# daigo0927/tf-raft

Measured on NVIDIA H100. Metric: frame-pairs/sec at 448×512 iters=12; final-flow max-abs vs ref, higher is better.
Workload: dtype f32

## Files before the change

tf_raft_b200/csrc/kernels.cuh:

```cuda
#pragma once
#include "common.cuh"

namespace raft {

__global__ void split_plane_kernel(const float* __restrict__ src, int src_stride, int src_c0, int nch, int nch_pad,
                                   __half* __restrict__ hi, __half* __restrict__ lo, int dst_stride, int dst_c0,
                                   size_t npix, float scale) {
  const size_t total = npix * (size_t)nch_pad;
  for (size_t i = blockIdx.x * (size_t)blockDim.x + threadIdx.x; i < total; i += (size_t)gridDim.x * blockDim.x) {
    const size_t px = i / nch_pad;
    const int c = (int)(i - px * nch_pad);
    __half h = __float2half_rn(0.f), l = h;
    if (c < nch) split_f16(src[px * src_stride + src_c0 + c] * scale, h, l);
    hi[px * dst_stride + dst_c0 + c] = h;
    lo[px * dst_stride + dst_c0 + c] = l;
  }
}

__global__ void avgpool2x2_kernel(const float* __restrict__ src, float* __restrict__ dst, size_t M, int H, int W,
                                  int C) {
  const int Ho = H / 2, Wo = W / 2;
  const size_t total = M * (size_t)Ho * Wo * C;
  for (size_t i = blockIdx.x * (size_t)blockDim.x + threadIdx.x; i < total; i += (size_t)gridDim.x * blockDim.x) {
    size_t t = i;
    const int c = (int)(t % C);
    t /= C;
    const int xo = (int)(t % Wo);
    t /= Wo;
    const int yo = (int)(t % Ho);
    const size_t m = t / Ho;
    const float* s = src + ((m * H + 2 * yo) * W + 2 * xo) * (size_t)C + c;
    const float a = s[0], b = s[C], cc = s[(size_t)W * C], d = s[(size_t)W * C + C];
    dst[i] = __fmul_rn(__fadd_rn(__fadd_rn(a, b), __fadd_rn(cc, d)), 0.25f);
  }
}

__global__ void coords_grid_kernel(float* __restrict__ out, int B, int h, int w) {
  const size_t total = (size_t)B * h * w;
  for (size_t i = blockIdx.x * (size_t)blockDim.x + threadIdx.x; i < total; i += (size_t)gridDim.x * blockDim.x) {
    const int x = (int)(i % w), y = (int)((i / w) % h);
    out[2 * i] = (float)x;
    out[2 * i + 1] = (float)y;
  }
}

struct TapGather { float c00, c01, c10, c11; int o00, o01, o10, o11; };
__device__ __forceinline__ TapGather tap_setup(int H, int W, float px, float py) {
  const float gx = fminf(fmaxf(px, 0.0f), (float)(W - 1));
  const float gy = fminf(fmaxf(py, 0.0f), (float)(H - 1));
  const float gx0 = floorf(gx), gx1 = ceilf(gx), gy0 = floorf(gy), gy1 = ceilf(gy);
  const float wy1 = __fsub_rn(gy1, gy), wy0 = __fsub_rn(gy, gy0);
  const float wx1 = __fsub_rn(gx1, gx), wx0 = __fsub_rn(gx, gx0);
  TapGather t;
  t.c00 = __fmul_rn(wy1, wx1); t.c01 = __fmul_rn(wy1, wx0);
  t.c10 = __fmul_rn(wy0, wx1); t.c11 = __fmul_rn(wy0, wx0);
  const int ix0 = (int)gx0, ix1 = (int)gx1, iy0 = (int)gy0, iy1 = (int)gy1;
  t.o00 = iy0 * W + ix0; t.o01 = iy0 * W + ix1; t.o10 = iy1 * W + ix0; t.o11 = iy1 * W + ix1;
  return t;
}
__device__ __forceinline__ float tap_combine(const TapGather& t, float x00, float x01, float x10, float x11) {
  float acc = __fmul_rn(t.c00, x00);
  acc = __fadd_rn(acc, __fmul_rn(t.c01, x01));
  acc = __fadd_rn(acc, __fmul_rn(t.c10, x10));
  acc = __fadd_rn(acc, __fmul_rn(t.c11, x11));
  return acc;
}
__device__ __forceinline__ float sample_floor_ceil(const float* __restrict__ img, int H, int W, float px, float py) {
  const TapGather t = tap_setup(H, W, px, py);
  return tap_combine(t, __ldg(img + t.o00), __ldg(img + t.o01), __ldg(img + t.o10), __ldg(img + t.o11));
}

__global__ void bilinear_sampler_kernel(const float* __restrict__ image, const float* __restrict__ coords, int M, int H,
                                        int W, int P, float* __restrict__ out) {
  const size_t total = (size_t)M * P;
  for (size_t i = blockIdx.x * (size_t)blockDim.x + threadIdx.x; i < total; i += (size_t)gridDim.x * blockDim.x) {
    const size_t m = i / P;
    out[i] = sample_floor_ceil(image + m * (size_t)H * W, H, W, coords[2 * i], coords[2 * i + 1]);
  }
}

struct LookupParams {
  const float* pyr[RAFT_MAX_LEVELS];
  int lh[RAFT_MAX_LEVELS], lw[RAFT_MAX_LEVELS];
  const float* coords;
  float* out; int out_stride;
  __half* out_hi; __half* out_lo; int h_stride, h_pad;
  int nq;
  int levels, radius;
  const float* im_flow; __half* im_hi; __half* im_lo; int im_B, im_h, im_w;
};

__global__ void __launch_bounds__(256) corr_lookup_kernel(const LookupParams p) {
  __shared__ float4 axis_smem[8 * 32];
  const int warps_per_block = blockDim.x >> 5;
  const int lane = threadIdx.x & 31;
  const int side = 2 * p.radius + 1, ntap = side * side;
  const size_t nwork = (size_t)p.nq * p.levels;
  for (size_t wi = (size_t)blockIdx.x * warps_per_block + (threadIdx.x >> 5); wi < nwork;
       wi += (size_t)gridDim.x * warps_per_block) {
    const int q = (int)(wi / p.levels), l = (int)(wi % p.levels);
    const int H = p.lh[l], W = p.lw[l];
    const float* img = p.pyr[l] + (size_t)q * H * W;
    const float inv = 1.0f / (float)(1 << l);
    const float cx = __fmul_rn(__ldg(p.coords + 2 * (size_t)q), inv);
    const float cy = __fmul_rn(__ldg(p.coords + 2 * (size_t)q + 1), inv);
    constexpr int kMaxIter = 3;
    if (ntap <= 32 * kMaxIter && side <= 16) {
      float4* ax = axis_smem + (threadIdx.x >> 5) * 32;
      __syncwarp();
      if (lane < 2 * side) {
        const bool isy = lane >= side;
        const int i = isy ? lane - side : lane;
        const float cc = isy ? cy : cx;
        const int dim = isy ? H : W;
        const float g = fminf(fmaxf(__fadd_rn(cc, (float)(i - p.radius)), 0.0f), (float)(dim - 1));
        const float g0 = floorf(g), g1 = ceilf(g);
        ax[(isy ? 16 : 0) + i] = make_float4(__fsub_rn(g1, g), __fsub_rn(g, g0), __int_as_float((int)g0), __int_as_float((int)g1));
      }
      __syncwarp();
      TapGather tg[kMaxIter];
      float x00[kMaxIter], x01[kMaxIter], x10[kMaxIter], x11[kMaxIter];
#pragma unroll
      for (int i = 0; i < kMaxIter; ++i) {
        const int t = min(lane + 32 * i, ntap - 1);
        const int a = t / side, b2 = t - a * side;
        const float4 sx = ax[a], sy = ax[16 + b2];
        const int ix0 = __float_as_int(sx.z), ix1 = __float_as_int(sx.w), iy0 = __float_as_int(sy.z), iy1 = __float_as_int(sy.w);
        tg[i].c00 = __fmul_rn(sy.x, sx.x); tg[i].c01 = __fmul_rn(sy.x, sx.y);
        tg[i].c10 = __fmul_rn(sy.y, sx.x); tg[i].c11 = __fmul_rn(sy.y, sx.y);
        x00[i] = __ldg(img + iy0 * W + ix0); x01[i] = __ldg(img + iy0 * W + ix1);
        x10[i] = __ldg(img + iy1 * W + ix0); x11[i] = __ldg(img + iy1 * W + ix1);
      }
#pragma unroll
      for (int i = 0; i < kMaxIter; ++i) {
        const int t = lane + 32 * i;
        if (t < ntap) {
          const float v = tap_combine(tg[i], x00[i], x01[i], x10[i], x11[i]);
          const int ch = l * ntap + t;
          if (p.out) p.out[(size_t)q * p.out_stride + ch] = v;
          if (p.out_hi) {
            __half hh, ll;
            split_f16(v, hh, ll);
            p.out_hi[(size_t)q * p.h_stride + ch] = hh;
            p.out_lo[(size_t)q * p.h_stride + ch] = ll;
          }
        }
      }
    } else {
      for (int t = lane; t < ntap; t += 32) {
        const int a = t / side, b2 = t - a * side;
        const float px = __fadd_rn(cx, (float)(a - p.radius));
        const float py = __fadd_rn(cy, (float)(b2 - p.radius));
        const float v = sample_floor_ceil(img, H, W, px, py);
        const int ch = l * ntap + t;
        if (p.out) p.out[(size_t)q * p.out_stride + ch] = v;
        if (p.out_hi) {
          __half hh, ll;
          split_f16(v, hh, ll);
          p.out_hi[(size_t)q * p.h_stride + ch] = hh;
          p.out_lo[(size_t)q * p.h_stride + ch] = ll;
        }
      }
    }
    if (p.out_hi && l == p.levels - 1) {
      const __half zero = __float2half_rn(0.f);
      for (int c = p.levels * ntap + lane; c < p.h_pad; c += 32) {
        p.out_hi[(size_t)q * p.h_stride + c] = zero;
        p.out_lo[(size_t)q * p.h_stride + c] = zero;
      }
    }
  }
}

__global__ void __launch_bounds__(256) corr_fp32_kernel(const float* __restrict__ f1, const float* __restrict__ f2,
                                                        float* __restrict__ out, int N, int C, float div) {
  __shared__ float As[16][64 + 4];
  __shared__ float Bs[16][64 + 4];
  const int b = blockIdx.z;
  const float* A = f1 + (size_t)b * N * C;
  const float* Bm = f2 + (size_t)b * N * C;
  float* O = out + (size_t)b * N * N;
  const int m0 = blockIdx.y * 64, n0 = blockIdx.x * 64;
  const int tx = threadIdx.x & 15, ty = threadIdx.x >> 4;
  const int lr = threadIdx.x >> 2, lc = (threadIdx.x & 3) * 4;
  float acc[4][4] = {};
  for (int k0 = 0; k0 < C; k0 += 16) {
#pragma unroll
    for (int j = 0; j < 4; ++j) {
      const int k = k0 + lc + j;
      As[lc + j][lr] = (m0 + lr < N && k < C) ? A[(size_t)(m0 + lr) * C + k] : 0.f;
      Bs[lc + j][lr] = (n0 + lr < N && k < C) ? Bm[(size_t)(n0 + lr) * C + k] : 0.f;
    }
    __syncthreads();
#pragma unroll
    for (int k = 0; k < 16; ++k) {
      float a[4], w[4];
#pragma unroll
      for (int i = 0; i < 4; ++i) {
        a[i] = As[k][ty * 4 + i];
        w[i] = Bs[k][tx * 4 + i];
      }
#pragma unroll
      for (int i = 0; i < 4; ++i)
#pragma unroll
        for (int j = 0; j < 4; ++j) acc[i][j] = fmaf(a[i], w[j], acc[i][j]);
    }
    __syncthreads();
  }
#pragma unroll
  for (int i = 0; i < 4; ++i)
#pragma unroll
    for (int j = 0; j < 4; ++j) {
      const int m = m0 + ty * 4 + i, n = n0 + tx * 4 + j;
      if (m < N && n < N) O[(size_t)m * N + n] = __fdiv_rn(acc[i][j], div);
    }
}

enum SimtAct : int { SACT_NONE = 0, SACT_RELU = 1, SACT_SIGMOID = 2, SACT_TANH = 3 };

struct SimtConvParams {
  const float* src[3]; int src_stride[3], src_c0[3], src_n[3]; int nsrc;
  const float* w; const float* bias;
  int kh, kw, cin, cout;
  int B, H, W;
  int stride, Hin, Win, pad_t, pad_l;
  int in_image_norm;
  const float* post_scale; const float* post_shift;
  float* out; int out_stride, out_c0;
  __half* out_hi; __half* out_lo; int h_stride, h_c0;
  int act; float out_scale;
};

__global__ void __launch_bounds__(256) conv_simt_kernel(const SimtConvParams p) {
  __shared__ float As[16][64 + 4];
  __shared__ float Ws[16][64 + 4];
  const int npix = p.B * p.H * p.W;
  const int m0 = blockIdx.x * 64, n0 = blockIdx.y * 64;
  const int tx = threadIdx.x & 15, ty = threadIdx.x >> 4;
  const int lr = threadIdx.x >> 2, lc = (threadIdx.x & 3) * 4;
  const int wr = threadIdx.x >> 4, wc = (threadIdx.x & 15) * 4;
  const int st = p.stride > 1 ? p.stride : 1;
  const int Hin = p.stride > 0 ? p.Hin : p.H, Win = p.stride > 0 ? p.Win : p.W;
  const int ph = p.stride > 0 ? p.pad_t : (p.kh - 1) / 2, pw = p.stride > 0 ? p.pad_l : (p.kw - 1) / 2;
  const int lp = m0 + lr;
  int lb = 0, ly = 0, lx = 0;
  if (lp < npix) {
    lx = lp % p.W;
    ly = (lp / p.W) % p.H;
    lb = lp / (p.W * p.H);
  }
  float acc[4][4] = {};
  for (int tap = 0; tap < p.kh * p.kw; ++tap) {
    const int dy = tap / p.kw - ph, dx = tap % p.kw - pw;
    const int sy = ly * st + dy, sx = lx * st + dx;
    const bool inb = lp < npix && sy >= 0 && sy < Hin && sx >= 0 && sx < Win;
    const size_t spix = ((size_t)lb * Hin + (inb ? sy : 0)) * Win + (inb ? sx : 0);
    for (int k0 = 0; k0 < p.cin; k0 += 16) {
#pragma unroll
      for (int j = 0; j < 4; ++j) {
        const int c = k0 + lc + j;
        float v = 0.f;
        if (inb && c < p.cin) {
          int cc = c, s = 0;
          while (s < p.nsrc - 1 && cc >= p.src_n[s]) cc -= p.src_n[s++];
          v = __ldg(p.src[s] + spix * p.src_stride[s] + p.src_c0[s] + cc);
          if (p.in_image_norm) v = __fsub_rn(__fmul_rn(2.0f, __fdiv_rn(v, 255.0f)), 1.0f);
        }
        As[lc + j][lr] = v;
      }
      {
        const int c = k0 + wr;
#pragma unroll
        for (int j = 0; j < 4; ++j) {
          const int n = n0 + wc + j;
          Ws[wr][wc + j] = (c < p.cin && n < p.cout) ? __ldg(p.w + ((size_t)tap * p.cin + c) * p.cout + n) : 0.f;
        }
      }
      __syncthreads();
#pragma unroll
      for (int k = 0; k < 16; ++k) {
        float a[4], w[4];
#pragma unroll
        for (int i = 0; i < 4; ++i) {
          a[i] = As[k][ty * 4 + i];
          w[i] = Ws[k][tx * 4 + i];
        }
#pragma unroll
        for (int i = 0; i < 4; ++i)
#pragma unroll
          for (int j = 0; j < 4; ++j) acc[i][j] = fmaf(a[i], w[j], acc[i][j]);
      }
      __syncthreads();
    }
  }
#pragma unroll
  for (int i = 0; i < 4; ++i) {
    const int m = m0 + ty * 4 + i;
    if (m >= npix) continue;
#pragma unroll
    for (int j = 0; j < 4; ++j) {
      const int n = n0 + tx * 4 + j;
      if (n >= p.cout) continue;
      float v = acc[i][j] + (p.bias ? __ldg(p.bias + n) : 0.f);
      if (p.post_scale) v = v * __ldg(p.post_scale + n) + __ldg(p.post_shift + n);
      if (p.act == SACT_RELU) v = relu_nan(v);
      else if (p.act == SACT_SIGMOID) v = sigmoidf_acc(v);
      else if (p.act == SACT_TANH) v = tanhf(v);
      v *= p.out_scale;
      if (p.out) p.out[(size_t)m * p.out_stride + p.out_c0 + n] = v;
      if (p.out_hi) {
        __half hh, ll;
        split_f16(v, hh, ll);
        p.out_hi[(size_t)m * p.h_stride + p.h_c0 + n] = hh;
        p.out_lo[(size_t)m * p.h_stride + p.h_c0 + n] = ll;
      }
    }
  }
}

__global__ void gru_rh_kernel(const float* __restrict__ r, const float* __restrict__ h, float* __restrict__ rh,
                              size_t n) {
  for (size_t i = blockIdx.x * (size_t)blockDim.x + threadIdx.x; i < n; i += (size_t)gridDim.x * blockDim.x)
    rh[i] = r[i] * h[i];
}
__global__ void gru_update_kernel(const float* __restrict__ z, const float* __restrict__ q, float* __restrict__ h,
                                  size_t n) {
  for (size_t i = blockIdx.x * (size_t)blockDim.x + threadIdx.x; i < n; i += (size_t)gridDim.x * blockDim.x)
    h[i] = (1.0f - z[i]) * h[i] + z[i] * q[i];
}

__global__ void copy_channels_kernel(const float* __restrict__ src, int src_stride, int src_c0,
                                     float* __restrict__ dst, int dst_stride, int dst_c0, int n, size_t npix) {
  const size_t total = npix * (size_t)n;
  for (size_t i = blockIdx.x * (size_t)blockDim.x + threadIdx.x; i < total; i += (size_t)gridDim.x * blockDim.x) {
    const size_t px = i / n;
    const int c = (int)(i - px * n);
    dst[px * dst_stride + dst_c0 + c] = src[px * src_stride + src_c0 + c];
  }
}

__global__ void flow_advance_kernel(float* __restrict__ coords1, const float* __restrict__ delta,
                                    float* __restrict__ flow, int B, int h, int w) {
  const size_t total = (size_t)B * h * w;
  for (size_t i = blockIdx.x * (size_t)blockDim.x + threadIdx.x; i < total; i += (size_t)gridDim.x * blockDim.x) {
    const float gx = (float)(i % w), gy = (float)((i / w) % h);
    float cx = coords1[2 * i], cy = coords1[2 * i + 1];
    if (delta) {
      cx = __fadd_rn(cx, delta[2 * i]);
      cy = __fadd_rn(cy, delta[2 * i + 1]);
      coords1[2 * i] = cx;
      coords1[2 * i + 1] = cy;
    }
    flow[2 * i] = __fsub_rn(cx, gx);
    flow[2 * i + 1] = __fsub_rn(cy, gy);
  }
}

__global__ void __launch_bounds__(256) upsample_convex_kernel(const float* __restrict__ flow,
                                                              const float* __restrict__ mask, int B, int h, int w,
                                                              float* __restrict__ out) {
  const int sub = threadIdx.x & 63;
  const size_t npix = (size_t)B * h * w;
  for (size_t pix = (size_t)blockIdx.x * 4 + (threadIdx.x >> 6); pix < npix; pix += (size_t)gridDim.x * 4) {
    const int x = (int)(pix % w), y = (int)((pix / w) % h), b = (int)(pix / ((size_t)w * h));
    const float* mp = mask + pix * 576 + sub * 9;
    float m[9], mx = -INFINITY;
#pragma unroll
    for (int k = 0; k < 9; ++k) {
      m[k] = __ldg(mp + k);
      mx = fmaxf(mx, m[k]);
    }
    float sum = 0.f;
#pragma unroll
    for (int k = 0; k < 9; ++k) {
      m[k] = expf(m[k] - mx);
      sum += m[k];
    }
    float ox = 0.f, oy = 0.f;
#pragma unroll
    for (int k = 0; k < 9; ++k) {
      const int yy = y + k / 3 - 1, xx = x + k % 3 - 1;
      float fx = 0.f, fy = 0.f;
      if (yy >= 0 && yy < h && xx >= 0 && xx < w) {
        const float* fp = flow + (((size_t)b * h + yy) * w + xx) * 2;
        fx = 8.0f * __ldg(fp);
        fy = 8.0f * __ldg(fp + 1);
      }
      const float wk = m[k] / sum;
      ox += wk * fx;
      oy += wk * fy;
    }
    const int by = sub >> 3, bx = sub & 7;
    float* op = out + ((((size_t)b * 8 * h) + 8 * y + by) * (8 * (size_t)w) + 8 * x + bx) * 2;
    *reinterpret_cast<float2*>(op) = make_float2(ox, oy);
  }
}

__global__ void upflow8_kernel(const float* __restrict__ flow, int B, int h, int w, float* __restrict__ out) {
  const int H = 8 * h, W = 8 * w;
  const size_t total = (size_t)B * H * W;
  for (size_t i = blockIdx.x * (size_t)blockDim.x + threadIdx.x; i < total; i += (size_t)gridDim.x * blockDim.x) {
    const int X = (int)(i % W), Y = (int)((i / W) % H), b = (int)(i / ((size_t)W * H));
    const float sx = ((float)X + 0.5f) * 0.125f - 0.5f, sy = ((float)Y + 0.5f) * 0.125f - 0.5f;
    const float fx0 = floorf(sx), fy0 = floorf(sy);
    const float ax = sx - fx0, ay = sy - fy0;
    const int x0 = min(max((int)fx0, 0), w - 1), x1 = min(max((int)fx0 + 1, 0), w - 1);
    const int y0 = min(max((int)fy0, 0), h - 1), y1 = min(max((int)fy0 + 1, 0), h - 1);
    const float* f = flow + (size_t)b * h * w * 2;
#pragma unroll
    for (int c = 0; c < 2; ++c) {
      const float v00 = f[((size_t)y0 * w + x0) * 2 + c], v01 = f[((size_t)y0 * w + x1) * 2 + c];
      const float v10 = f[((size_t)y1 * w + x0) * 2 + c], v11 = f[((size_t)y1 * w + x1) * 2 + c];
      const float top = v00 * (1.f - ax) + v01 * ax, bot = v10 * (1.f - ax) + v11 * ax;
      out[2 * i + c] = 8.0f * (top * (1.f - ay) + bot * ay);
    }
  }
}

__global__ void absmax_kernel(const float* __restrict__ w, size_t n, unsigned int* __restrict__ out_bits) {
  float m = 0.f;
  for (size_t i = blockIdx.x * (size_t)blockDim.x + threadIdx.x; i < n; i += (size_t)gridDim.x * blockDim.x)
    m = fmaxf(m, fabsf(w[i]));
  for (int o = 16; o > 0; o >>= 1) m = fmaxf(m, __shfl_xor_sync(0xffffffffu, m, o));
  if ((threadIdx.x & 31) == 0) atomicMax(out_bits, __float_as_uint(m));
}

__global__ void weight_scale_kernel(const unsigned int* __restrict__ absmax_bits, float* __restrict__ scale) {
  const float m = __uint_as_float(*absmax_bits);
  int k = 0;
  if (m > 0.f && isfinite(m)) {
    int e;
    frexpf(m, &e);
    k = 13 - e;
    k = max(-24, min(24, k));
  }
  scale[0] = ldexpf(1.0f, k);
  scale[1] = ldexpf(1.0f, -k);
}

struct PackParams {
  const float* w; int kh, kw, cin, cout;
  __half* hi; __half* lo; int cout_pad, cin_pad, cout_off;
  int r_src0[2], r_n[2], r_dst0[2], nrange;
  const float* scale;
};
__global__ void pack_weights_kernel(const PackParams p) {
  const size_t total = (size_t)p.kh * p.kw * p.cin * p.cout;
  const float s = p.scale[0];
  for (size_t i = blockIdx.x * (size_t)blockDim.x + threadIdx.x; i < total; i += (size_t)gridDim.x * blockDim.x) {
    size_t t = i;
    const int n = (int)(t % p.cout);
    t /= p.cout;
    const int c = (int)(t % p.cin);
    const int tap = (int)(t / p.cin);
    int cd = -1;
    for (int r = 0; r < p.nrange; ++r)
      if (c >= p.r_src0[r] && c < p.r_src0[r] + p.r_n[r]) cd = p.r_dst0[r] + (c - p.r_src0[r]);
    if (cd < 0) continue;
    __half hh, ll;
    split_f16(p.w[i] * s, hh, ll);
    const size_t o = ((size_t)tap * p.cout_pad + p.cout_off + n) * p.cin_pad + cd;
    p.hi[o] = hh;
    p.lo[o] = ll;
  }
}

constexpr int kNormBlock = 8;
__device__ __forceinline__ void chan_merge(float& na, float& ma, float& m2a, float nb, float mb, float m2b) {
  if (nb == 0.f) return;
  const float n = na + nb, d = mb - ma;
  ma = ma + d * (nb / n);
  m2a = m2a + m2b + d * d * (na * nb / n);
  na = n;
}
__global__ void __launch_bounds__(256) norm_stats_kernel(const float* __restrict__ y, int P, int C, int nsplit,
                                                         float* __restrict__ part) {
  __shared__ float red[3][256];
  const int g = blockIdx.x, sp = blockIdx.y;
  const int lanes = 256 / C > 0 ? 256 / C : 1;
  const int c = threadIdx.x % C, pl = threadIdx.x / C;
  const int per = (P + nsplit - 1) / nsplit;
  const int p0 = sp * per, p1 = min(P, p0 + per);
  float n = 0.f, mean = 0.f, m2 = 0.f;
  if (pl < lanes && p0 + pl < p1) {
    const float* base = y + ((size_t)g * P) * C + c;
    mean = base[(size_t)(p0 + pl) * C];
    n = 1.f;
    for (int px = p0 + pl + lanes; px < p1;) {
      float s1 = 0.f, s2 = 0.f;
#pragma unroll
      for (int k = 0; k < kNormBlock; ++k, px += lanes) {
        if (px < p1) {
          const float v = base[(size_t)px * C] - mean;
          s1 += v;
          s2 += v * v;
          n += 1.f;
        }
      }
      const float r = s1 / n;
      mean += r;
      m2 += relu_nan(s2 - s1 * r);
    }
  }
  red[0][threadIdx.x] = n; red[1][threadIdx.x] = mean; red[2][threadIdx.x] = m2;
  __syncthreads();
  if (pl == 0) {
    for (int l = 1; l < lanes; ++l) chan_merge(n, mean, m2, red[0][l * C + c], red[1][l * C + c], red[2][l * C + c]);
    float* o = part + (((size_t)g * nsplit + sp) * 3) * C + c;
    o[0] = n; o[C] = mean; o[2 * C] = m2;
  }
}
__global__ void norm_final_kernel(const float* __restrict__ part, int G, int C, int nsplit,
                                  const float* __restrict__ gamma, float eps, float* __restrict__ mean_out,
                                  float* __restrict__ mult_out) {
  const int i = (blockIdx.x * blockDim.x + threadIdx.x) >> 5, lane = threadIdx.x & 31;
  if (i >= G * C) return;
  const int g = i / C, c = i % C;
  float n = 0.f, mean = 0.f, m2 = 0.f;
  for (int s = lane; s < nsplit; s += 32) {
    const float* o = part + (((size_t)g * nsplit + s) * 3) * C + c;
    chan_merge(n, mean, m2, o[0], o[C], o[2 * C]);
  }
#pragma unroll
  for (int off = 16; off > 0; off >>= 1) {
    const float nb = __shfl_xor_sync(0xffffffffu, n, off), mb = __shfl_xor_sync(0xffffffffu, mean, off),
                m2b = __shfl_xor_sync(0xffffffffu, m2, off);
    float na = n, ma = mean, m2a = m2;
    if (lane & off) { na = nb; ma = mb; m2a = m2b; chan_merge(na, ma, m2a, n, mean, m2); }
    else chan_merge(na, ma, m2a, nb, mb, m2b);
    n = na; mean = ma; m2 = m2a;
  }
  if (lane == 0) {
    mean_out[i] = mean;
    mult_out[i] = rsqrtf(m2 / n + eps) * gamma[c];
  }
}
__global__ void norm_apply_kernel(const float* __restrict__ y, size_t npix, int P, int C, int per_image,
                                  const float* __restrict__ mean, const float* __restrict__ a,
                                  const float* __restrict__ beta, int relu, const float* __restrict__ skip32,
                                  const __half* __restrict__ skip_hi, const __half* __restrict__ skip_lo,
                                  float* __restrict__ out32, __half* __restrict__ hi, __half* __restrict__ lo,
                                  int c_pad) {
  const int gpp = c_pad >> 3;
  const size_t total = npix * (size_t)gpp;
  for (size_t i = blockIdx.x * (size_t)blockDim.x + threadIdx.x; i < total; i += (size_t)gridDim.x * blockDim.x) {
    const size_t px = i / gpp;
    const int c = (int)(i - px * gpp) << 3;
    float v[8] = {0.f, 0.f, 0.f, 0.f, 0.f, 0.f, 0.f, 0.f};
    if (c < C) {
      const size_t g = per_image ? px / P : 0;
      const float* yp = y + px * C + c;
      const float* mp = mean + g * C + c;
      const float* ap = a + g * C + c;
      const float* bp = beta + c;
      float4 t[2] = {*reinterpret_cast<const float4*>(yp), *reinterpret_cast<const float4*>(yp + 4)};
      const float yy[8] = {t[0].x, t[0].y, t[0].z, t[0].w, t[1].x, t[1].y, t[1].z, t[1].w};
#pragma unroll
      for (int e = 0; e < 8; ++e) {
        v[e] = (yy[e] - __ldg(mp + e)) * __ldg(ap + e) + __ldg(bp + e);
        if (relu) v[e] = relu_nan(v[e]);
      }
      if (skip32) {
        const float4 s0 = *reinterpret_cast<const float4*>(skip32 + px * C + c), s1 = *reinterpret_cast<const float4*>(skip32 + px * C + c + 4);
        const float ss[8] = {s0.x, s0.y, s0.z, s0.w, s1.x, s1.y, s1.z, s1.w};
#pragma unroll
        for (int e = 0; e < 8; ++e) v[e] = relu_nan(ss[e] + v[e]);
      } else if (skip_hi) {
        const uint4 h4 = *reinterpret_cast<const uint4*>(skip_hi + px * c_pad + c), l4 = *reinterpret_cast<const uint4*>(skip_lo + px * c_pad + c);
        const uint32_t hw[4] = {h4.x, h4.y, h4.z, h4.w}, lw[4] = {l4.x, l4.y, l4.z, l4.w};
#pragma unroll
        for (int e = 0; e < 4; ++e) {
          const float2 hf = __half22float2(*reinterpret_cast<const __half2*>(&hw[e]));
          const float2 lf = __half22float2(*reinterpret_cast<const __half2*>(&lw[e]));
          v[2 * e] = relu_nan(hf.x + lf.x + v[2 * e]);
          v[2 * e + 1] = relu_nan(hf.y + lf.y + v[2 * e + 1]);
        }
      }
      if (out32) {
        *reinterpret_cast<float4*>(out32 + px * C + c) = make_float4(v[0], v[1], v[2], v[3]);
        *reinterpret_cast<float4*>(out32 + px * C + c + 4) = make_float4(v[4], v[5], v[6], v[7]);
      }
    }
    if (hi) {
      uint32_t ph[4], pl[4];
#pragma unroll
      for (int e = 0; e < 4; ++e) split_f16x2(v[2 * e], v[2 * e + 1], ph[e], pl[e]);
      *reinterpret_cast<uint4*>(hi + px * c_pad + c) = make_uint4(ph[0], ph[1], ph[2], ph[3]);
      *reinterpret_cast<uint4*>(lo + px * c_pad + c) = make_uint4(pl[0], pl[1], pl[2], pl[3]);
    }
  }
}
__global__ void image_norm_kernel(const float* __restrict__ img, float* __restrict__ out, size_t n) {
  for (size_t i = blockIdx.x * (size_t)blockDim.x + threadIdx.x; i < n; i += (size_t)gridDim.x * blockDim.x)
    out[i] = __fsub_rn(__fmul_rn(2.0f, __fdiv_rn(img[i], 255.0f)), 1.0f);
}

__global__ void stem_im2col_kernel(const float* __restrict__ img, int N, int H, int W, int h, int w, int pad_t,
                                   int pad_l, int image_norm, __half* __restrict__ hi, __half* __restrict__ lo) {
  const size_t total = (size_t)N * h * w * 24;
  for (size_t i = blockIdx.x * (size_t)blockDim.x + threadIdx.x; i < total; i += (size_t)gridDim.x * blockDim.x) {
    const int grp = (int)(i % 24);
    const size_t px = i / 24;
    const int x = (int)(px % w), y = (int)((px / w) % h), n = (int)(px / ((size_t)w * h));
    uint32_t ph[4] = {0u, 0u, 0u, 0u}, pl[4] = {0u, 0u, 0u, 0u};
    if (grp * 8 < 147) {
      int ty = (grp * 8) / 21, j = grp * 8 - ty * 21;
      const int ix0 = 2 * x - pad_l;
      const float* base = img + ((size_t)n * H * W + ix0) * 3;
      float v[8];
#pragma unroll
      for (int e = 0; e < 8; ++e) {
        const int iy = 2 * y + ty - pad_t, ix = ix0 + ((j * 11) >> 5);
        v[e] = 0.f;
        if (ty < 7 && iy >= 0 && iy < H && ix >= 0 && ix < W) {
          v[e] = __ldg(base + (ptrdiff_t)iy * W * 3 + j);
          if (image_norm) v[e] = __fsub_rn(__fmul_rn(2.0f, __fdiv_rn(v[e], 255.0f)), 1.0f);
        }
        if (++j == 21) { j = 0; ++ty; }
      }
#pragma unroll
      for (int e = 0; e < 4; ++e) split_f16x2(v[2 * e], v[2 * e + 1], ph[e], pl[e]);
    }
    reinterpret_cast<uint4*>(hi)[i] = make_uint4(ph[0], ph[1], ph[2], ph[3]);
    reinterpret_cast<uint4*>(lo)[i] = make_uint4(pl[0], pl[1], pl[2], pl[3]);
  }
}

__device__ __forceinline__ void flow_im2col_rider(const float* __restrict__ flow, int B, int h, int w, __half* __restrict__ hi,
                                                  __half* __restrict__ lo, size_t tid, size_t nthreads) {
  const size_t total = (size_t)B * h * w * 16;
  for (size_t i = tid; i < total; i += nthreads) {
    const int g = (int)(i & 15);
    const size_t px = i >> 4;
    const int x = (int)(px % w), y = (int)((px / w) % h);
    uint32_t ph[4], pl[4];
#pragma unroll
    for (int e = 0; e < 4; ++e) {
      const int tap = 4 * g + e;
      float2 v = make_float2(0.f, 0.f);
      if (tap < 49) {
        const int yy = y + tap / 7 - 3, xx = x + tap % 7 - 3;
        if (yy >= 0 && yy < h && xx >= 0 && xx < w)
          v = __ldg(reinterpret_cast<const float2*>(flow) + (ptrdiff_t)px + (ptrdiff_t)(yy - y) * w + (xx - x));
      }
      split_f16x2(v.x, v.y, ph[e], pl[e]);
    }
    reinterpret_cast<uint4*>(hi)[i] = make_uint4(ph[0], ph[1], ph[2], ph[3]);
    reinterpret_cast<uint4*>(lo)[i] = make_uint4(pl[0], pl[1], pl[2], pl[3]);
  }
}

__global__ void flow_im2col_kernel(const float* __restrict__ flow, int B, int h, int w, __half* __restrict__ hi,
                                   __half* __restrict__ lo) {
  const size_t total = (size_t)B * h * w * 128;
  for (size_t i = blockIdx.x * (size_t)blockDim.x + threadIdx.x; i < total; i += (size_t)gridDim.x * blockDim.x) {
    const int kk = (int)(i & 127);
    const size_t px = i >> 7;
    float v = 0.f;
    if (kk < 98) {
      const int x = (int)(px % w), y = (int)((px / w) % h);
      const int tap = kk >> 1, c = kk & 1;
      const int yy = y + tap / 7 - 3, xx = x + tap % 7 - 3;
      if (yy >= 0 && yy < h && xx >= 0 && xx < w) v = __ldg(flow + (px + (size_t)(yy - y) * w + (xx - x)) * 2 + c);
    }
    __half hh, ll;
    split_f16(v, hh, ll);
    hi[i] = hh;
    lo[i] = ll;
  }
}

__global__ void bn_fold_kernel(const float* __restrict__ gamma, const float* __restrict__ beta,
                               const float* __restrict__ mean, const float* __restrict__ var, float eps, int C,
                               float* __restrict__ scale, float* __restrict__ shift) {
  const int c = blockIdx.x * blockDim.x + threadIdx.x;
  if (c >= C) return;
  const float s = gamma[c] * rsqrtf(var[c] + eps);
  scale[c] = s;
  shift[c] = beta[c] - mean[c] * s;
}
__global__ void context_split_kernel(const float* __restrict__ cnet, size_t npix, int hid, int ctx,
                                     float* __restrict__ net, float* __restrict__ inp) {
  const int C = hid + ctx;
  const size_t total = npix * (size_t)C;
  for (size_t i = blockIdx.x * (size_t)blockDim.x + threadIdx.x; i < total; i += (size_t)gridDim.x * blockDim.x) {
    const size_t px = i / C;
    const int c = (int)(i - px * C);
    const float v = cnet[i];
    if (c < hid) net[px * hid + c] = tanhf(v);
    else inp[px * ctx + (c - hid)] = relu_nan(v);
  }
}

inline int grid_for(size_t n, int block = 256, int cap = kNumSMs * 16) {
  size_t g = (n + block - 1) / block;
  if (g < 1) g = 1;
  if (g > (size_t)cap) g = cap;
  return (int)g;
}

}
```

tf_raft_b200/layers/extractor.py:

```python
import ctypes
import math
import os

import torch
import torch.nn.functional as F

from .. import _lib


def force_ieee_fp32():
    try:
        torch.backends.cudnn.conv.fp32_precision = 'ieee'
        torch.backends.cuda.matmul.fp32_precision = 'ieee'
    except Exception:
        torch.backends.cudnn.allow_tf32 = False
        torch.backends.cuda.matmul.allow_tf32 = False


force_ieee_fp32()


def _same_pads(n_in, k, s):
    n_out = -(-n_in // s)
    total = max((n_out - 1) * s + k - n_in, 0)
    return total // 2, total - total // 2


def _glorot(shape, gen):
    kh, kw, cin, cout = shape
    limit = math.sqrt(6.0 / (kh * kw * cin + kh * kw * cout))
    return torch.empty(shape).uniform_(-limit, limit, generator=gen)


class _Params:

    def __init__(self, device):
        self.device = torch.device(device)
        self.params = {}
        self._nchw_cache = {}

    def add_conv(self, name, kh, kw, cin, cout, gen):
        self.params[name + '.kernel'] = _glorot((kh, kw, cin, cout), gen).to(self.device)
        self.params[name + '.bias'] = torch.zeros(cout, device=self.device)

    def add_norm(self, name, norm_type, c):
        if norm_type is None:
            return
        self.params[name + '.gamma'] = torch.ones(c, device=self.device)
        self.params[name + '.beta'] = torch.zeros(c, device=self.device)
        if norm_type == 'batch':
            self.params[name + '.moving_mean'] = torch.zeros(c, device=self.device)
            self.params[name + '.moving_variance'] = torch.ones(c, device=self.device)

    def load(self, params, prefix=''):
        for name in self.params:
            src = torch.as_tensor(params[prefix + name], dtype=torch.float32)
            if tuple(src.shape) != tuple(self.params[name].shape):
                raise ValueError(f'{prefix + name}: expected {tuple(self.params[name].shape)}, got {tuple(src.shape)}')
            self.params[name] = src.to(self.device).contiguous()
        self._nchw_cache.clear()

    def conv(self, x, name, stride=1, padding='same'):
        w = self._nchw_cache.get(name)
        if w is None:
            w = self.params[name + '.kernel'].permute(3, 2, 0, 1).contiguous()
            self._nchw_cache[name] = w
        if padding == 'same':
            pt, pb = _same_pads(x.shape[2], w.shape[2], stride)
            pl, pr = _same_pads(x.shape[3], w.shape[3], stride)
            if pt or pb or pl or pr:
                x = F.pad(x, (pl, pr, pt, pb))
        return F.conv2d(x, w, self.params[name + '.bias'], stride=stride)

    def norm(self, x, name, norm_type, training):
        eps = 1e-3
        if norm_type is None:
            return x
        g = self.params[name + '.gamma'].view(1, -1, 1, 1)
        b = self.params[name + '.beta'].view(1, -1, 1, 1)
        if norm_type == 'instance':
            mean = x.mean(dim=(2, 3), keepdim=True)
            var = x.var(dim=(2, 3), unbiased=False, keepdim=True)
        elif norm_type == 'batch':
            if training:
                mean = x.mean(dim=(0, 2, 3), keepdim=True)
                var = x.var(dim=(0, 2, 3), unbiased=False, keepdim=True)
                mom, n = 0.99, x.shape[0] * x.shape[2] * x.shape[3]
                self.params[name + '.moving_mean'].mul_(mom).add_((1 - mom) * mean.flatten())
                self.params[name + '.moving_variance'].mul_(mom).add_((1 - mom) * n / max(n - 1, 1) * var.flatten())
            else:
                mean = self.params[name + '.moving_mean'].view(1, -1, 1, 1)
                var = self.params[name + '.moving_variance'].view(1, -1, 1, 1)
        else:
            raise ValueError(f'Invalid norm_type specified: {norm_type}')
        return (x - mean) * torch.rsqrt(var + eps) * g + b


def Normalization(norm_type, groups=None):
    if norm_type in ('batch', 'instance', None):
        return norm_type
    if norm_type == 'group':
        raise NotImplementedError('GroupNormalization is not used by RAFT / SmallRAFT')
    raise ValueError(f'Invalid norm_type specified: {norm_type}')


class _Encoder:
    _c0 = 0
    _stages = ()
    _variant = None

    def __init__(self, output_dim=128, norm_type='batch', drop_rate=0.0, *, device='cuda', seed=None, backend=None):
        self.backend = backend or os.environ.get('RAFT_B200_ENCODER', 'native')
        if self.backend not in ('native', 'torch'):
            raise ValueError(f'unknown encoder backend {self.backend!r}')
        self._prepared = None
        self._ws = {}
        self.output_dim = output_dim
        self.norm_type = Normalization(norm_type)
        self.drop_rate = drop_rate
        gen = torch.Generator(device='cpu')
        gen.manual_seed(0 if seed is None else seed)
        self.store = _Params(device)
        s = self.store
        s.add_conv('conv1', 7, 7, 3, self._c0, gen)
        s.add_norm('norm1', norm_type, self._c0)
        cin = self._c0
        for li, (c, stride) in enumerate(self._stages, start=1):
            for bi, st in enumerate((stride, 1)):
                p = f'layer{li}.{bi}'
                s.add_conv(p + '.conv1', 3, 3, cin, c, gen)
                s.add_conv(p + '.conv2', 3, 3, c, c, gen)
                s.add_norm(p + '.norm1', norm_type, c)
                s.add_norm(p + '.norm2', norm_type, c)
                if st != 1:
                    s.add_conv(p + '.downsample.0', 1, 1, cin, c, gen)
                    s.add_norm(p + '.downsample.1', norm_type, c)
                cin = c
        s.add_conv('conv2', 1, 1, cin, output_dim, gen)

    @property
    def params(self):
        return self.store.params

    def load_params(self, params, prefix=''):
        self.store.load(params, prefix)
        self._prepared = None

    def state_dict(self, prefix=''):
        return {prefix + k: v for k, v in self.store.params.items()}

    def _conv_struct(self, name):
        k = self.store.params[name + '.kernel']
        return _lib.RaftConv(k.data_ptr(), self.store.params[name + '.bias'].data_ptr(), *k.shape)

    def _norm_struct(self, name):
        p = self.store.params
        if self.norm_type is None:
            return _lib.RaftNorm(None, None, None, None)
        mm = p.get(name + '.moving_mean')
        mv = p.get(name + '.moving_variance')
        return _lib.RaftNorm(p[name + '.gamma'].data_ptr(), p[name + '.beta'].data_ptr(),
                             None if mm is None else mm.data_ptr(), None if mv is None else mv.data_ptr())

    def prepared(self):
        if self._prepared is None:
            L = _lib.lib()
            w = _lib.RaftEncoderWeights()
            w.conv1 = self._conv_struct('conv1')
            w.norm1 = self._norm_struct('norm1')
            k = 0
            for li, (_, stride) in enumerate(self._stages, start=1):
                for bi, st in enumerate((stride, 1)):
                    p = f'layer{li}.{bi}'
                    blk = w.block[k]
                    blk.conv1, blk.conv2 = self._conv_struct(p + '.conv1'), self._conv_struct(p + '.conv2')
                    blk.norm1, blk.norm2 = self._norm_struct(p + '.norm1'), self._norm_struct(p + '.norm2')
                    if st != 1:
                        blk.downsample = self._conv_struct(p + '.downsample.0')
                        blk.downsample_norm = self._norm_struct(p + '.downsample.1')
                    k += 1
            w.conv2 = self._conv_struct('conv2')
            nbytes = ctypes.c_size_t()
            _lib.check(L.raft_b200_encoder_prepared_bytes(self._variant, self.output_dim, ctypes.byref(nbytes)),
                       'encoder_prepared_bytes')
            blob = _lib.workspace(nbytes.value, self.store.device)
            with torch.cuda.device(self.store.device):
                _lib.check(L.raft_b200_encoder_prepare(self._variant, _lib.NORM_TYPES[self.norm_type], self.output_dim,
                                                       ctypes.cast(ctypes.pointer(w), ctypes.c_void_p), _lib.ptr(blob),
                                                       blob.numel(), _lib.stream()), 'encoder_prepare')
            self._prepared = blob
        return self._prepared

    def _native(self, x, training, raw_image):
        x = _lib.f32c(x)
        n, h, w, c = x.shape
        if c != 3:
            raise ValueError(f'encoder input must be (N, H, W, 3); got {tuple(x.shape)}')
        L = _lib.lib()
        key = (n, h, w)
        if key not in self._ws:
            nbytes = ctypes.c_size_t()
            _lib.check(L.raft_b200_encoder_workspace_bytes(self._variant, n, h, w, ctypes.byref(nbytes)),
                       'encoder_workspace_bytes')
            self._ws = {key: _lib.workspace(nbytes.value, x.device)}
        ws = self._ws[key]
        out = torch.empty((n, -(-h // 8), -(-w // 8), self.output_dim), dtype=torch.float32, device=x.device)
        with torch.cuda.device(x.device):
            _lib.check(L.raft_b200_encoder_forward(self._variant, _lib.NORM_TYPES[self.norm_type], self.output_dim,
                                                   _lib.ptr(self.prepared()), _lib.ptr(x), n, h, w, int(bool(training)),
                                                   int(bool(raw_image)), _lib.ptr(out), _lib.ptr(ws), ws.numel(),
                                                   _lib.stream()), 'encoder_forward')
        return out

    def _res_block(self, x, p, stride, training):
        s, nt = self.store, self.norm_type
        fx = F.relu(s.norm(s.conv(x, p + '.conv1', stride), p + '.norm1', nt, training))
        fx = F.relu(s.norm(s.conv(fx, p + '.conv2', 1), p + '.norm2', nt, training))
        if stride != 1:
            x = s.norm(s.conv(x, p + '.downsample.0', stride, padding='valid'), p + '.downsample.1', nt, training)
        return F.relu(x + fx)

    def __call__(self, inputs, training=False, *, raw_image=False):
        is_list = isinstance(inputs, (tuple, list))
        x = torch.cat(list(inputs), dim=0) if is_list else inputs
        if self.backend == 'native' and not (self.drop_rate > 0 and training):
            out = self._native(x, training, raw_image)
            if is_list:
                n = out.shape[0] // 2
                return [out[:n], out[n:]]
            return out
        if raw_image:
            x = 2 * (x / 255.0) - 1.0
        x = x.permute(0, 3, 1, 2)
        s, nt = self.store, self.norm_type
        x = F.relu(s.norm(s.conv(x, 'conv1', 2), 'norm1', nt, training))
        for li, (_, stride) in enumerate(self._stages, start=1):
            x = self._res_block(x, f'layer{li}.0', stride, training)
            x = self._res_block(x, f'layer{li}.1', 1, training)
        x = s.conv(x, 'conv2', 1, padding='valid')
        if self.drop_rate > 0 and training:
            x = F.dropout(x, self.drop_rate, training=True)
        x = x.permute(0, 2, 3, 1).contiguous()
        if is_list:
            n = x.shape[0] // 2
            return [x[:n].contiguous(), x[n:].contiguous()]
        return x


class BasicEncoder(_Encoder):
    _c0 = 64
    _stages = ((64, 1), (96, 2), (128, 2))
    _variant = _lib.VARIANT_BASIC


class SmallEncoder(_Encoder):
    _c0 = 32
    _stages = ((32, 1), (64, 2), (96, 2))
    _variant = _lib.VARIANT_SMALL
```

tf_raft_b200/model.py:

```python
from collections import OrderedDict

import torch

from . import _lib
from .layers.corr import CorrBlock, coords_grid, coords_init, fb_occlusion, forward_interpolate, upflow8
from .layers.extractor import BasicEncoder, SmallEncoder
from .layers.update import BasicUpdateBlock, SmallUpdateBlock
from .losses import end_point_error, sequence_loss


class RAFT:
    _variant = _lib.VARIANT_BASIC

    def __init__(self, drop_rate=0, iters=12, iters_pred=24, *, precision=None, device='cuda', seed=None,
                 use_graph=False, encoder_backend=None, **kwargs):
        self.hidden_dim = 128
        self.context_dim = 128
        self.corr_levels = 4
        self.corr_radius = 4
        self.drop_rate = drop_rate
        self.iters = iters
        self.iters_pred = iters_pred
        self.precision = _lib.resolve_precision(precision)
        self.device = torch.device(device)
        self.use_graph = use_graph
        self.encoder_backend = encoder_backend
        self._build_layers(seed)
        self._graphs = {}
        self.flow_metrics = None
        self.optimizer = None
        self._trainer = None
        self._params_stale = False

    def _encoder_backend(self):
        return self.encoder_backend or ('native' if self.precision == _lib.PREC_F16X2 else 'torch')

    def _build_layers(self, seed):
        s = 0 if seed is None else seed
        self.fnet = BasicEncoder(output_dim=256, norm_type='instance', drop_rate=self.drop_rate, device=self.device,
                                 seed=s, backend=self._encoder_backend())
        self.cnet = BasicEncoder(output_dim=self.hidden_dim + self.context_dim, norm_type='batch',
                                 drop_rate=self.drop_rate, device=self.device, seed=s + 1, backend=self._encoder_backend())
        self.update_block = BasicUpdateBlock(filters=self.hidden_dim, precision=self.precision, device=self.device,
                                             seed=s + 2)

    def load_params(self, params):
        self.fnet.load_params(params, 'fnet.')
        self.cnet.load_params(params, 'cnet.')
        self.update_block.load_params(params, 'update_block.')
        self._graphs.clear()
        self._trainer = None
        self._params_stale = False

    def state_dict(self):
        self._sync_trained_params()
        out = OrderedDict()
        out.update(self.fnet.state_dict('fnet.'))
        out.update(self.cnet.state_dict('cnet.'))
        out.update(self.update_block.state_dict('update_block.'))
        return out

    def initialize_flow(self, image):
        bs, h, w, _ = image.shape
        return coords_grid(bs, h // 8, w // 8, self.device), coords_grid(bs, h // 8, w // 8, self.device)

    def upsample_flow(self, flow, mask):
        flow, mask = _lib.f32c(flow), _lib.f32c(mask)
        b, h, w, _ = flow.shape
        if tuple(mask.shape) != (b, h, w, 576):
            raise ValueError(f'mask: expected {(b, h, w, 576)}, got {tuple(mask.shape)}')
        out = torch.empty((b, 8 * h, 8 * w, 2), dtype=torch.float32, device=flow.device)
        with torch.cuda.device(flow.device):
            _lib.check(_lib.lib().raft_b200_upsample_convex(_lib.ptr(flow), _lib.ptr(mask), b, h, w, _lib.ptr(out),
                                                            _lib.stream()), 'upsample_convex')
        return out

    def _encode(self, image1, image2, training):
        fmap1, fmap2 = self.fnet([image1, image2], training=training, raw_image=True)
        net, inp = self._context(image1, training)
        return fmap1, fmap2, net, inp

    def _context(self, image1, training):
        cnet = self.cnet(image1, training=training, raw_image=True)
        b, h, w, _ = cnet.shape
        net = torch.empty((b, h, w, self.hidden_dim), dtype=torch.float32, device=cnet.device)
        inp = torch.empty((b, h, w, self.context_dim), dtype=torch.float32, device=cnet.device)
        with torch.cuda.device(cnet.device):
            _lib.check(_lib.lib().raft_b200_context_split(_lib.ptr(cnet), b * h * w, self.hidden_dim,
                                                          self.context_dim, _lib.ptr(net), _lib.ptr(inp),
                                                          _lib.stream()), 'context_split')
        return net, inp

    def _loop(self, corr_block, net, inp, coords1, flow_ups, b, h, w):
        ub = self.update_block
        ws = ub.workspace(b, h, w)
        with torch.cuda.device(self.device):
            _lib.check(_lib.lib().raft_b200_forward_loop(
                self._variant, _lib.ptr(ub.prepared()), _lib.ptr_array(corr_block.corr_pyramid), self.corr_levels,
                self.corr_radius, _lib.ptr(net), _lib.ptr(inp), _lib.ptr(coords1), _lib.ptr_array(flow_ups),
                len(flow_ups), b, h, w, _lib.ptr(ws), ws.numel(), self.precision, _lib.stream()), 'forward_loop')

    def __call__(self, inputs, training, *, last_only=False, flow_init=None):
        image1, image2 = inputs
        image1, image2 = _lib.f32c(image1), _lib.f32c(image2)
        if flow_init is not None:
            flow_init = self._check_flow_init(flow_init, image1)
        self._sync_trained_params()
        if self.use_graph and not training:
            key = (tuple(image1.shape), bool(last_only), flow_init is not None)
            return self._graph_run(key, lambda a, b, f: self._forward(a, b, False, last_only, f),
                                   (image1, image2, flow_init))
        return self._forward(image1, image2, training, last_only, flow_init)

    @staticmethod
    def _check_flow_init(flow_init, image):
        if not isinstance(flow_init, torch.Tensor):
            raise TypeError(f'flow_init must be a torch tensor, got {type(flow_init).__name__}')
        if flow_init.dtype != torch.float32:
            raise TypeError(f'flow_init must be float32, got {flow_init.dtype}')
        if flow_init.device != image.device:
            raise ValueError(f'flow_init is on {flow_init.device}, the images on {image.device}')
        bs, H, W, _ = image.shape
        want = (bs, H // 8, W // 8, 2)
        if tuple(flow_init.shape) != want:
            raise ValueError(f'flow_init: expected {want} for {H}x{W} images, got {tuple(flow_init.shape)}')
        return flow_init.contiguous()

    def _graph_run(self, key, fn, inputs):
        entry = self._graphs.get(key)
        if entry is None:
            statics = [None if t is None else t.clone() for t in inputs]
            side = torch.cuda.Stream(device=self.device)
            side.wait_stream(torch.cuda.current_stream(self.device))
            with torch.cuda.stream(side):
                for _ in range(2):
                    fn(*statics)
            torch.cuda.current_stream(self.device).wait_stream(side)
            torch.cuda.synchronize(self.device)
            graph = torch.cuda.CUDAGraph()
            with torch.cuda.graph(graph):
                outs = fn(*statics)
            keep = [list(m._ws.values()) for m in (self.fnet, self.cnet, self.update_block)]
            entry = (graph, statics, outs, self._last, keep)
            self._graphs[key] = entry
        graph, statics, outs, last, _keep = entry
        for s, t in zip(statics, inputs):
            if t is not None:
                s.copy_(t, non_blocking=True)
        graph.replay()
        self._last = last
        return outs

    @staticmethod
    def _check_size(H, W):
        if H % 8 or W % 8:
            raise ValueError(f'image height and width must be multiples of 8 (got {H}x{W}); the reference fails in '
                             'update.py:146 for other sizes -- crop-or-pad first (datasets/dataset.py:323-334)')

    def _forward(self, image1, image2, training, last_only, flow_init=None):
        bs, H, W, _ = image1.shape
        self._check_size(H, W)
        fmap1, fmap2, net, inp = self._encode(image1, image2, training)
        return self._iterate(fmap1, fmap2, net, inp, bs, H, W, training, last_only, flow_init)

    def _iterate(self, fmap1, fmap2, net, inp, bs, H, W, training, last_only, flow_init):
        h, w = H // 8, W // 8
        iters = self.iters if training else self.iters_pred
        corr_block = CorrBlock(fmap1, fmap2, num_levels=self.corr_levels, radius=self.corr_radius,
                               precision=self.precision)
        if flow_init is None:
            coords1 = coords_grid(bs, h, w, self.device)
        else:
            coords1 = coords_init(flow_init)
        preds = [torch.empty((bs, H, W, 2), dtype=torch.float32, device=self.device)
                 if (not last_only or i == iters - 1) else None for i in range(iters)]
        if iters:
            self._loop(corr_block, net, inp, coords1, preds, bs, h, w)
        self._last = dict(net=net, coords1=coords1, corr_block=corr_block)
        return [p for p in preds if p is not None] if last_only else preds

    def predict_bidirectional(self, inputs):
        image1, image2 = inputs
        image1, image2 = _lib.f32c(image1), _lib.f32c(image2)
        if image1.shape != image2.shape:
            raise ValueError(f'image1 {tuple(image1.shape)} and image2 {tuple(image2.shape)} differ in shape')
        if self.iters_pred < 1:
            raise ValueError('predict_bidirectional needs iters_pred >= 1')
        self._sync_trained_params()
        if self.use_graph:
            return self._graph_run(('bidirectional', tuple(image1.shape)), self._bidirectional, (image1, image2))
        return self._bidirectional(image1, image2)

    def _bidirectional(self, image1, image2):
        bs, H, W, _ = image1.shape
        self._check_size(H, W)
        images = torch.cat([image1, image2])
        fmap = self.fnet(images, training=False, raw_image=True)
        net, inp = self._context(images, False)
        return self._iterate_bidirectional(fmap, torch.cat([fmap[bs:], fmap[:bs]]), net, inp, bs, H, W, None)

    def _iterate_bidirectional(self, fmap1, fmap2, net, inp, bs, H, W, flow_init):
        flow = self._iterate(fmap1, fmap2, net, inp, 2 * bs, H, W, False, True, flow_init)[-1]
        flow_fw, flow_bw = flow[:bs], flow[bs:]
        return (flow_fw, flow_bw) + fb_occlusion(flow_fw, flow_bw)

    def predict_video(self, frames, *, warm_start=True, bidirectional=False):
        self._sync_trained_params()
        if self.iters_pred < 1:
            raise ValueError('predict_video needs iters_pred >= 1')
        shape = coords0 = frame_prev = fmap_prev = flow_init = ctx_prev = None
        for t, frame in enumerate(frames):
            frame = _lib.f32c(frame)
            if shape is None:
                shape = tuple(frame.shape)
                if len(shape) != 4 or shape[-1] != 3:
                    raise ValueError(f'frames must be (B, H, W, 3); got {shape}')
                bs, H, W, _ = shape
                self._check_size(H, W)
            elif tuple(frame.shape) != shape:
                raise ValueError(f'frame {t}: shape {tuple(frame.shape)} differs from the first frame {shape}')
            fmap = self.fnet(frame, training=False, raw_image=True)
            if bidirectional:
                ctx = self._context(frame, False)
            if frame_prev is not None:
                if bidirectional:
                    net, inp = (torch.cat([p, c]) for p, c in zip(ctx_prev, ctx))
                    out = self._iterate_bidirectional(torch.cat([fmap_prev, fmap]), torch.cat([fmap, fmap_prev]), net,
                                                      inp, bs, H, W, flow_init)
                else:
                    net, inp = self._context(frame_prev, False)
                    out = self._iterate(fmap_prev, fmap, net, inp, bs, H, W, False, True, flow_init)[-1]
                if warm_start:
                    if coords0 is None:
                        coords0 = coords_grid(2 * bs if bidirectional else bs, H // 8, W // 8, self.device)
                    if bidirectional:
                        flow_low = self._last['coords1'] - coords0
                        flow_low[bs:].neg_()
                        flow_init = forward_interpolate(flow_low)
                        flow_init[bs:].neg_()
                    else:
                        flow_init = forward_interpolate(self._last['coords1'] - coords0)
                yield out
            frame_prev, fmap_prev = frame, fmap
            if bidirectional:
                ctx_prev = ctx

    call = __call__

    def compile(self, optimizer=None, clip_norm=None, loss=sequence_loss, epe=end_point_error, **kwargs):
        self.optimizer = optimizer
        self.clip_norm = clip_norm
        self.loss = loss
        self.epe = epe
        self.flow_metrics = OrderedDict((k, [0.0, 0]) for k in ('loss', 'epe', 'u1', 'u3', 'u5'))

    def _metric_update(self, key, value):
        m = self.flow_metrics[key]
        m[0] += float(value)
        m[1] += 1

    def _metric_results(self):
        return {k: (s / n if n else 0.0) for k, (s, n) in self.flow_metrics.items()}

    def train_step(self, data):
        from .train import AdamW, Trainer
        if self.flow_metrics is None or getattr(self, 'optimizer', None) is None:
            raise RuntimeError('compile(optimizer=..., clip_norm=...) before train_step, as in train_chairs.py:92-98')
        if not isinstance(self.optimizer, AdamW):
            raise TypeError('optimizer must be tf_raft_b200.train.AdamW (tfa.optimizers.AdamW semantics)')
        if self._trainer is None:
            self._trainer = Trainer(self)
        loss, info = self._trainer.step(data, self.optimizer, self.clip_norm, self.loss, self.epe)
        self._params_stale = True
        self._metric_update('loss', loss)
        for k in ('epe', 'u1', 'u3', 'u5'):
            self._metric_update(k, info[k])
        return self._metric_results()

    def _sync_trained_params(self):
        if self._trainer is not None and self._params_stale:
            trainer = self._trainer
            self.load_params(trainer.params())
            self._trainer = trainer
            self._params_stale = False

    def test_step(self, data):
        if self.flow_metrics is None:
            self.compile()
        image1, image2, flow, valid = data
        preds = self([image1, image2], training=False, last_only=True)
        info = self.epe([flow, valid], preds[-1])
        for k in ('epe', 'u1', 'u3', 'u5'):
            self._metric_update(k, info[k])
        return self._metric_results()

    def predict_step(self, data):
        image1, image2, *_ = data
        return self([image1, image2], training=False, last_only=True)[-1]

    def reset_metrics(self):
        if self.flow_metrics is not None:
            for m in self.flow_metrics.values():
                m[0], m[1] = 0.0, 0


class SmallRAFT(RAFT):
    _variant = _lib.VARIANT_SMALL

    def _build_layers(self, seed):
        self.hidden_dim = 96
        self.context_dim = 64
        self.corr_levels = 4
        self.corr_radius = 3
        s = 0 if seed is None else seed
        self.fnet = SmallEncoder(output_dim=128, norm_type='instance', drop_rate=self.drop_rate, device=self.device,
                                 seed=s, backend=self._encoder_backend())
        self.cnet = SmallEncoder(output_dim=self.hidden_dim + self.context_dim, norm_type=None,
                                 drop_rate=self.drop_rate, device=self.device, seed=s + 1, backend=self._encoder_backend())
        self.update_block = SmallUpdateBlock(filters=self.hidden_dim, precision=self.precision, device=self.device,
                                             seed=s + 2)

    def upsample_flow(self, flow, mask=None):
        return upflow8(flow)
```

Baseline: 310.5.

## Overlap context encoder on side stream, prefetch norm stats, 32-bit im2col indexing

In inference mode the context encoder now runs on a separate CUDA stream so it overlaps with the feature encoder, with stream waits and record_stream calls to keep memory safe. The encoder workspace setup is pulled into its own method so it can be allocated before the side stream launches. The norm-stats kernel software-pipelines its strided loads by prefetching the next block into registers. The stem im2col kernel uses 32-bit index arithmetic when the range fits, avoiding 64-bit divisions. Risks: a second stream adds synchronisation and can contend for SMs, and the prefetch raises register use.

Result: faster. 318.5, median of 6 (+2.6%).

```diff
diff --git a/tf_raft_b200/csrc/kernels.cuh b/tf_raft_b200/csrc/kernels.cuh
--- a/tf_raft_b200/csrc/kernels.cuh
+++ b/tf_raft_b200/csrc/kernels.cuh
@@ -486,17 +486,31 @@
     const float* base = y + ((size_t)g * P) * C + c;
     mean = base[(size_t)(p0 + pl) * C];
     n = 1.f;
-    for (int px = p0 + pl + lanes; px < p1;) {
+    const int step = kNormBlock * lanes;
+    float nxt[kNormBlock];
+    int px = p0 + pl + lanes;
+#pragma unroll
+    for (int k = 0; k < kNormBlock; ++k) nxt[k] = px + k * lanes < p1 ? base[(size_t)(px + k * lanes) * C] : 0.f;
+    while (px < p1) {
+      float cur[kNormBlock];
+#pragma unroll
+      for (int k = 0; k < kNormBlock; ++k) cur[k] = nxt[k];
+      if (px + step < p1) {
+#pragma unroll
+        for (int k = 0; k < kNormBlock; ++k)
+          nxt[k] = px + step + k * lanes < p1 ? base[(size_t)(px + step + k * lanes) * C] : 0.f;
+      }
       float s1 = 0.f, s2 = 0.f;
 #pragma unroll
-      for (int k = 0; k < kNormBlock; ++k, px += lanes) {
-        if (px < p1) {
-          const float v = base[(size_t)px * C] - mean;
+      for (int k = 0; k < kNormBlock; ++k) {
+        if (px + k * lanes < p1) {
+          const float v = cur[k] - mean;
           s1 += v;
           s2 += v * v;
           n += 1.f;
         }
       }
+      px += step;
       const float r = s1 / n;
       mean += r;
       m2 += relu_nan(s2 - s1 * r);
@@ -595,13 +609,14 @@
     out[i] = __fsub_rn(__fmul_rn(2.0f, __fdiv_rn(img[i], 255.0f)), 1.0f);
 }
 
-__global__ void stem_im2col_kernel(const float* __restrict__ img, int N, int H, int W, int h, int w, int pad_t,
-                                   int pad_l, int image_norm, __half* __restrict__ hi, __half* __restrict__ lo) {
-  const size_t total = (size_t)N * h * w * 24;
-  for (size_t i = blockIdx.x * (size_t)blockDim.x + threadIdx.x; i < total; i += (size_t)gridDim.x * blockDim.x) {
+template <class I>
+__device__ __forceinline__ void stem_im2col_body(const float* __restrict__ img, int N, int H, int W, int h, int w, int pad_t,
+                                                 int pad_l, int image_norm, __half* __restrict__ hi, __half* __restrict__ lo) {
+  const I total = (I)N * h * w * 24;
+  for (I i = blockIdx.x * (I)blockDim.x + threadIdx.x; i < total; i += (I)gridDim.x * blockDim.x) {
     const int grp = (int)(i % 24);
-    const size_t px = i / 24;
-    const int x = (int)(px % w), y = (int)((px / w) % h), n = (int)(px / ((size_t)w * h));
+    const I px = i / 24;
+    const int x = (int)(px % w), y = (int)((px / w) % h), n = (int)(px / ((I)w * h));
     uint32_t ph[4] = {0u, 0u, 0u, 0u}, pl[4] = {0u, 0u, 0u, 0u};
     if (grp * 8 < 147) {
       int ty = (grp * 8) / 21, j = grp * 8 - ty * 21;
@@ -625,6 +640,12 @@
     reinterpret_cast<uint4*>(lo)[i] = make_uint4(pl[0], pl[1], pl[2], pl[3]);
   }
 }
+__global__ void stem_im2col_kernel(const float* __restrict__ img, int N, int H, int W, int h, int w, int pad_t,
+                                   int pad_l, int image_norm, __half* __restrict__ hi, __half* __restrict__ lo) {
+  const size_t total = (size_t)N * h * w * 24, stride = (size_t)gridDim.x * blockDim.x;
+  if (total + stride <= 0xFFFFFFFFull) stem_im2col_body<unsigned int>(img, N, H, W, h, w, pad_t, pad_l, image_norm, hi, lo);
+  else stem_im2col_body<size_t>(img, N, H, W, h, w, pad_t, pad_l, image_norm, hi, lo);
+}
 
 __device__ __forceinline__ void flow_im2col_rider(const float* __restrict__ flow, int B, int h, int w, __half* __restrict__ hi,
                                                   __half* __restrict__ lo, size_t tid, size_t nthreads) {
diff --git a/tf_raft_b200/layers/extractor.py b/tf_raft_b200/layers/extractor.py
--- a/tf_raft_b200/layers/extractor.py
+++ b/tf_raft_b200/layers/extractor.py
@@ -191,19 +191,22 @@
             self._prepared = blob
         return self._prepared
 
+    def workspace(self, n, h, w, device):
+        key = (n, h, w)
+        if key not in self._ws:
+            nbytes = ctypes.c_size_t()
+            _lib.check(_lib.lib().raft_b200_encoder_workspace_bytes(self._variant, n, h, w, ctypes.byref(nbytes)),
+                       'encoder_workspace_bytes')
+            self._ws = {key: _lib.workspace(nbytes.value, device)}
+        return self._ws[key]
+
     def _native(self, x, training, raw_image):
         x = _lib.f32c(x)
         n, h, w, c = x.shape
         if c != 3:
             raise ValueError(f'encoder input must be (N, H, W, 3); got {tuple(x.shape)}')
         L = _lib.lib()
-        key = (n, h, w)
-        if key not in self._ws:
-            nbytes = ctypes.c_size_t()
-            _lib.check(L.raft_b200_encoder_workspace_bytes(self._variant, n, h, w, ctypes.byref(nbytes)),
-                       'encoder_workspace_bytes')
-            self._ws = {key: _lib.workspace(nbytes.value, x.device)}
-        ws = self._ws[key]
+        ws = self.workspace(n, h, w, x.device)
         out = torch.empty((n, -(-h // 8), -(-w // 8), self.output_dim), dtype=torch.float32, device=x.device)
         with torch.cuda.device(x.device):
             _lib.check(L.raft_b200_encoder_forward(self._variant, _lib.NORM_TYPES[self.norm_type], self.output_dim,
diff --git a/tf_raft_b200/model.py b/tf_raft_b200/model.py
--- a/tf_raft_b200/model.py
+++ b/tf_raft_b200/model.py
@@ -76,9 +76,33 @@
         return out
 
     def _encode(self, image1, image2, training):
+        if training:
+            fmap1, fmap2 = self.fnet([image1, image2], training=training, raw_image=True)
+            net, inp = self._context(image1, training)
+            return fmap1, fmap2, net, inp
+        main = torch.cuda.current_stream(image1.device)
+        side = self._encode_stream(image1.device)
+        if self.cnet.backend == 'native':
+            self.cnet.prepared()
+            self.cnet.workspace(*image1.shape[:3], image1.device)
+        side.wait_stream(main)
+        with torch.cuda.stream(side):
+            net, inp = self._context(image1, training)
         fmap1, fmap2 = self.fnet([image1, image2], training=training, raw_image=True)
-        net, inp = self._context(image1, training)
+        main.wait_stream(side)
+        if not torch.cuda.is_current_stream_capturing():
+            image1.record_stream(side)
+            net.record_stream(main)
+            inp.record_stream(main)
         return fmap1, fmap2, net, inp
+
+    def _encode_stream(self, device):
+        s = getattr(self, '_side_streams', None)
+        if s is None:
+            s = self._side_streams = {}
+        if device not in s:
+            s[device] = torch.cuda.Stream(device=device)
+        return s[device]
 
     def _context(self, image1, training):
         cnet = self.cnet(image1, training=training, raw_image=True)
```
